# CICE-Consortium/CICE

Measured on AMD Instinct MI355X. Metric: EVP subcycle cell-updates/sec (gx1 fp64), higher is better.
Workload: dtype f64

## Files before the change

### cice_amd/csrc/evp_host_resident.cpp

```cpp
#include "evp_host.h"
#include "rim_plan.h"

namespace evp_host {

bool tripole_seam() { return (S.n_seam + S.n_pole + S.n_late) > 0 || S.plan.tail > 0 || !S.plan.fin_dst.empty(); }

static bool tfold_image(size_t k)
{
    if (!S.plan.tfold) return false;
    const int dst = S.plan.local_dst[k];
    const int b = dst / (int)S.plane, r = dst % (int)S.plane, j = r / S.d.nx_block + 1, i = r % S.d.nx_block + 1;
    return i >= S.ilo[b] && i <= S.ihi[b] && j >= S.jlo[b] && j <= S.jhi[b];
}

bool resident_possible(bool with_peers)
{
    if (!with_peers && !S.plan.peers.empty()) return false;
    if (S.plan.tfold) {
        for (const HaloPeer &p : S.plan.peers)
            for (int k = 0; k < p.n_ghost_recv; ++k) {
                const int dst = p.recv_dst[k];
                const int b = dst / (int)S.plane, r = dst % (int)S.plane, j = r / S.d.nx_block + 1, i = r % S.d.nx_block + 1;
                if (i >= S.ilo[b] && i <= S.ihi[b] && j >= S.jlo[b] && j <= S.jhi[b]) return false;
            }
// ... 176 lines not shown
        }
    if (!S.res_err) {
        if (S.mem.alloc(S.res_err, 8)) return -1;
        HIPC(hipMemset(S.res_err, 0, 8 * sizeof(int)));
    }
    return 0;
}

bool resident2_fits(bool remote)
{
    struct Key { int dev, logw, strict, capm; unsigned fl; bool remote; long cap; };
    static std::vector<Key> known;
    const unsigned fl = S.flags & S.flags_allowed & ~(EVP_F_WATER_IS_OCN | EVP_F_TBU_ZERO);
    long cap = -1;
    for (const Key &k : known)
        if (k.dev == S.device && k.logw == S.res2_logw && k.strict == (S.prm.strict != 0) && k.capm == cap_mode() && k.fl == fl && k.remote == remote)
            cap = k.cap;
    if (cap < 0) {
        hipDeviceProp_t prop;
        if (hipGetDeviceProperties(&prop, S.device) != hipSuccess) return false;
        const int per_cu = std::min(evp_resident2_max_blocks_per_cu(S.prm.strict != 0, cap_mode(), fl, S.res2_logw, remote), 8);
        cap = (long)per_cu * prop.multiProcessorCount;
        known.push_back(Key{S.device, S.res2_logw, S.prm.strict != 0, cap_mode(), fl, remote, cap});
    }
    const int need = (remote || !S.plan.peers.empty() || S.res2_order_stale || !S.res2_order || S.res2_order_for != S.res2_logw)
                         ? S.res2_ntiles : std::max(S.res2_nlive, 1);
    return S.res2_ntiles > 0 && (long)need * 10 <= cap * 9;
}


bool resident2_fits_now()
{
    if (!S.plan.peers.empty() || S.res_remote) return true;
    if (resident_tables() || resident2_order()) { g_err.clear(); return false; }
    return resident2_fits(false);
}

int resident2_order()
{
    if (S.res2_order && !S.res2_order_stale && S.res2_order_for == S.res2_logw) return 0;
    const int W = 1 << S.res2_logw, H = 256 / W;
    int gx, gy;
    evp_resident_geometry(S.max_ni, S.max_nj, S.res2_logw, &gx, &gy);
    const int ntiles = gx * gy * S.d.nblocks, nx = S.d.nx_block;
    const bool permuted = !S.res2_cls_h.empty() && S.res2_logw == 4;
    std::vector<int> cost((size_t)ntiles);
    std::vector<uint8_t> live((size_t)ntiles, 1);
    std::vector<uint8_t> perm(permuted ? (size_t)ntiles * 256 : 0), late(permuted ? (size_t)ntiles : 0),
                         nact(permuted ? (size_t)ntiles : 0), nlt(permuted ? (size_t)ntiles : 0);
    bool coop_ok = permuted;
    const bool rim = permuted && S.d.nblocks == 1;
    std::vector<uint8_t> perm_rim(rim ? (size_t)ntiles * 256 : 0), uperm(rim ? (size_t)ntiles * 256 : 0), nact_rim(rim ? (size_t)ntiles : 0);
    bool rimu_ok = rim;
    for (int t = 0; t < ntiles; ++t) {
        const int b = t / (gx * gy), bx = (t % (gx * gy)) % gx, by = (t % (gx * gy)) / gx;
        const int i0 = S.ilo[b] + bx * (W - 1), j0 = S.jlo[b] + by * (H - 1);
        auto ice = [&](int pos) -> bool {
            const int i = i0 + (pos & (W - 1)), j = j0 + pos / W;
            if (i > S.ihi[b] + 1 || j > S.jhi[b] + 1) return false;
            return (S.hmask[b * S.plane + (size_t)(j - 1) * nx + (i - 1)] & 3u) != 0;
        };
        int n = 0, waves = 0;
        if (permuted) {
            const uint8_t *cl = &S.res2_cls_h[(size_t)t * 256];
            uint8_t *pm = &perm[(size_t)t * 256];
            int k = 0, nlate = 0;
            for (int pass = 0; pass < 3; ++pass)
                for (int pos = 0; pos < 256; ++pos) {
                    const bool on = cl[pos] != 0 && ice(pos);
                    const int which = on ? (cl[pos] == 2 ? 0 : 1) : 2;
                    if (which != pass) continue;
                    pm[k++] = (uint8_t)pos;
                    if (pass == 0) ++nlate;
                    if (pass < 2) ++n;
                }
            waves = (n + 63) / 64;
            nact[t] = (uint8_t)waves;
            late[t] = (uint8_t)std::min(4, (std::max(nlate, S.res2_cnt_h[t]) + 63) / 64);
            nlt[t] = (uint8_t)std::min(n, 64);
            if (nlate > 64) coop_ok = false;
            if (rim) {
                uint8_t icep[256], uown[256], upub[256];
                for (int pos = 0; pos < 256; ++pos) {
                    const int i = i0 + (pos & (W - 1)), j = j0 + pos / W;
                    icep[pos] = ice(pos);
                    uown[pos] = (pos & (W - 1)) < W - 1 && pos / W < H - 1 && i <= S.ihi[b] && j <= S.jhi[b];
                    upub[pos] = uown[pos] && S.res2_pubimg_h[b * S.plane + (size_t)(j - 1) * nx + (i - 1)];
                }
                rim_plan::Tile rt;
                rim_plan::tile(cl, icep, uown, upub, rt);
                std::copy(rt.perm, rt.perm + 256, &perm_rim[(size_t)t * 256]);
                std::copy(rt.uperm, rt.uperm + 256, &uperm[(size_t)t * 256]);
                nact_rim[t] = (uint8_t)rt.nact;
                if (!rt.ok || late[t] > 1) rimu_ok = false;
                waves = std::max(waves, rt.nact);
            }
        } else {
            int wave_on[4] = {0, 0, 0, 0};
            for (int pos = 0; pos < 256; ++pos)
                if (ice(pos)) { ++n; wave_on[pos >> 6] = 1; }
            waves = wave_on[0] + wave_on[1] + wave_on[2] + wave_on[3];
        }
        cost[t] = 1024 * waves + n;
        const bool no_ucell = i0 > S.ihi[b] || j0 > S.jhi[b];
        live[t] = !no_ucell && (n > 0 || S.res2_always_h[t] || !S.plan.peers.empty()) ? 1 : 0;
        if (no_ucell && env_test("CICE_EVP_HIP_RES_DEBUG") && (std::atoi(env_test("CICE_EVP_HIP_RES_DEBUG")) & 512)) live[t] = 1;
// ... 257 lines not shown
```

### cice_amd/csrc/evp_resident2.hip

```cpp
#include <hip/hip_runtime.h>
#include <stdint.h>
#include <algorithm>
#include <type_traits>

#ifdef CICE_EVP_HIP_TESTING
#define RES_DBG(R) ((R).dbg)
#define RES_PROF(R) ((R).prof != nullptr)
#else
#define RES_DBG(R) 0
#define RES_PROF(R) false
#endif

#include "evp_math.h"

namespace {

constexpr int RTY = 4;

typedef unsigned v4u __attribute__((ext_vector_type(4)));

__device__ __forceinline__ void st_rec2(void *p, v4u a, v4u b)
{
    asm volatile("global_store_dwordx4 %0, %1, off sc1\n\tglobal_store_dwordx4 %0, %2, off offset:16 sc1"
                 :
// ... 40 lines not shown
    const unsigned long long bits = (unsigned long long)__double_as_longlong(x);
    v4u r;
    r.x = tag; r.y = (unsigned)bits; r.z = (unsigned)(bits >> 32); r.w = tag;
    return r;
}
__device__ __forceinline__ double unpack_rec(v4u r)
{
    return __longlong_as_double((long long)(((unsigned long long)r.z << 32) | r.y));
}

template <int CTRL>
__device__ __forceinline__ double quad_perm(double v)
{
    const long long b = __double_as_longlong(v);
    const int lo = __builtin_amdgcn_update_dpp(0, (int)(b & 0xffffffffll), CTRL, 0xf, 0xf, false);
    const int hi = __builtin_amdgcn_update_dpp(0, (int)(b >> 32), CTRL, 0xf, 0xf, false);
    return __longlong_as_double(((long long)hi << 32) | (unsigned)lo);
}
constexpr int QP_X1 = 0xB1, QP_X2 = 0x4E, QP_X3 = 0x1B;

template <bool STRICT, int CAP, int LOGW, bool REMOTE, bool COOP = false, bool LEAN = false, bool RIMU = false>
__global__ __launch_bounds__(64 * RTY, REMOTE ? 2 : 3) void evp_resident2_tile(EvpArgs A, EvpResident2 R)
{
    static_assert(!COOP || (STRICT && CAP == 3 && LOGW == 4), "COOP: 16 x 16 tiles, strict build, default scalars");
    static_assert(!LEAN || (!REMOTE && !COOP && LOGW == 4), "LEAN: one rank, 16 x 16 tiles, one thread per rim cell");
    static_assert(!RIMU || LEAN, "RIMU: a schedule of the lean loop");
    using MM = Math<STRICT>;
#ifdef CICE_EVP_HIP_TESTING
    constexpr bool RANGE = LEAN;
#else
    constexpr bool RANGE = LEAN && EVP_RES2_RANGE_DEFAULT;
#endif
    using POL = std::conditional_t<RANGE, std::conditional_t<RIMU, evp_range::RangeMathLazy, evp_range::RangeMath>, evp_range::LibMath>;
    using POLE = std::conditional_t<RANGE, evp_range::RangeMath, evp_range::LibMath>;
    constexpr int W = 1 << LOGW;
    constexpr int H = 256 / W;
    constexpr int LW = W + 1;
    constexpr int NUV = ((H + 1) * LW + 7) & ~7;
    constexpr bool PERM = (LOGW == 4);
    constexpr int NSTR = RIMU ? 8 : PERM ? 6 : 4;
    constexpr int SW = PERM ? W + 1 : W;
    constexpr int SP = SW * H;
    extern __shared__ __attribute__((aligned(16))) double smem[];
    double *s_str = smem;
    double *s_tc = smem + NSTR * SP;
    double *s_u = s_tc + 4 * 256;
    double *s_v = s_u + NUV;
    double *s_uc = s_v + NUV;
    double *s_rc = nullptr, *s_r04 = nullptr;
    __shared__ int s_bad;

    __shared__ int s_chunk[4], s_simd[4], s_cu;
    __shared__ int s_slot[4];

    const int tx = threadIdx.x, ty = threadIdx.y;
    const int t = ty * 64 + tx;
    const int tile = R.order ? R.order[blockIdx.x] : (int)blockIdx.x;
    bool no_ucell;
    {
        const int pb = A.gx * A.gy;
        const int4 rb = A.blk[tile / pb];
        no_ucell = rb.x + ((tile % pb) % A.gx) * (W - 1) > rb.y || rb.z + ((tile % pb) / A.gx) * (H - 1) > rb.w;
        if (no_ucell && !(RES_DBG(R) & 512)) return;
    }
    int tq = t;
    int cu_rank = 0;
    if (PERM && R.cuload && !(RES_DBG(R) & 64)) {
        const int wave = t >> 6;
        if ((t & 63) == 0) {
            unsigned hw, xcc;
            asm volatile("s_getreg_b32 %0, hwreg(HW_REG_HW_ID)" : "=s"(hw));
            asm volatile("s_getreg_b32 %0, hwreg(HW_REG_XCC_ID)" : "=s"(xcc));
            s_simd[wave] = (int)((hw >> 4) & 3u);
            if (wave == 0) s_cu = (int)(((xcc & 7u) << 8) | ((hw >> 8) & 0xffu));
        }
        __syncthreads();
        if (t == 0) {
            int *L = R.cuload + 8 * s_cu;
            const int nact = R.nact[tile];
            int chunk_of[4] = {0, 1, 2, 3};
            unsigned spins = 0;
            bool locked = false;
            while (spins++ < 200000u) {
                if (atomicCAS(&L[0], 0, 1) == 0) { locked = true; break; }
                __builtin_amdgcn_s_sleep(2);
            }
            if (locked) {
                int ld[4];
                const int stamp = __hip_atomic_load(&L[1], __ATOMIC_RELAXED, __HIP_MEMORY_SCOPE_AGENT);
                const bool fresh = stamp != (int)R.tag_base;
#pragma unroll
                for (int q = 0; q < 4; ++q)
                    ld[q] = fresh ? 0 : __hip_atomic_load(&L[2 + q], __ATOMIC_RELAXED, __HIP_MEMORY_SCOPE_AGENT);
                const int rank = fresh ? 0 : __hip_atomic_load(&L[6], __ATOMIC_RELAXED, __HIP_MEMORY_SCOPE_AGENT);
                s_simd[0] |= rank << 8;
                bool used[4] = {false, false, false, false};
                for (int ck = 0; ck < 4; ++ck) {
                    int best = -1;
                    for (int w = 0; w < 4; ++w) {
                        if (used[w]) continue;
                        if (best < 0 || ld[s_simd[w] & 3] < ld[s_simd[best] & 3]) best = w;
                    }
                    used[best] = true;
                    chunk_of[best] = ck;
                    if (ck < nact) ld[s_simd[best] & 3] += 1;
                }
#pragma unroll
                for (int q = 0; q < 4; ++q) __hip_atomic_store(&L[2 + q], ld[q], __ATOMIC_RELAXED, __HIP_MEMORY_SCOPE_AGENT);
                __hip_atomic_store(&L[6], rank + 1, __ATOMIC_RELAXED, __HIP_MEMORY_SCOPE_AGENT);
                __hip_atomic_store(&L[1], (int)R.tag_base, __ATOMIC_RELAXED, __HIP_MEMORY_SCOPE_AGENT);
                asm volatile("s_waitcnt vmcnt(0)" ::: "memory");
                __hip_atomic_store(&L[0], 0, __ATOMIC_RELAXED, __HIP_MEMORY_SCOPE_AGENT);
            }
#pragma unroll
            for (int w = 0; w < 4; ++w) s_chunk[w] = chunk_of[w];
        }
        __syncthreads();
        tq = s_chunk[wave] * 64 + (t & 63);
        cu_rank = s_simd[0] >> 8;
    }
    const int pos = PERM ? (int)R.perm[tile * 256 + tq] : t;
    const int tcol = pos & (W - 1);
    const int trow = pos >> LOGW;
    const int sp = trow * SW + tcol;
    const int late_waves = PERM ? (int)R.late_waves[tile] : 4;
    const bool split = PERM && late_waves <= 1 && !(RES_DBG(R) & 32);
    if ((RES_DBG(R) & 16) && tile == 1 && !R.dry) return;
    const int per_blk = A.gx * A.gy;
    const int bz = tile / per_blk;
    const int bx = (tile % per_blk) % A.gx;
    const int by = (tile % per_blk) / A.gx;
    const int4 r = A.blk[bz];
    const int i0 = r.x + bx * (W - 1), j0 = r.z + by * (H - 1);
    const int i = i0 + tcol;
    const int j = j0 + trow;
    const int nx = A.nx, ny = A.ny;
    const int cb = bz * (int)A.plane;
    const int c = cb + (j - 1) * nx + (i - 1);
    const int li = (trow + 1) * LW + (tcol + 1);
    const int upos = RIMU ? (int)R.uperm[tile * 256 + tq] : pos;
    const int ucol = upos & (W - 1), urow = upos >> LOGW;
    const int ui = RIMU ? i0 + ucol : i, uj = RIMU ? j0 + urow : j;
    const int cu = RIMU ? cb + (uj - 1) * nx + (ui - 1) : c;
    const int uli = RIMU ? (urow + 1) * LW + (ucol + 1) : li;
    const int usp = RIMU ? urow * SW + ucol : sp;
    const unsigned flags = A.flags;
    const bool water = !LEAN && !(flags & EVP_F_WATER_IS_OCN);
    const bool tbu = !LEAN && !(flags & EVP_F_TBU_ZERO);
    if (COOP) {
        s_rc = s_uc + (8 + (water ? 2 : 0) + (tbu ? 1 : 0)) * 256;
        s_r04 = s_rc + 10 * 64;
    }

    const bool inT = (i <= r.y + 1) && (j <= r.w + 1);
    unsigned m = 0;
    if (inT) m = A.mask[c];
    const bool actT = inT && (m & 1u);
    const bool ownU = (ucol < W - 1) && (urow < H - 1) && (ui <= r.y) && (uj <= r.w);
    unsigned mU = m;
    if (RIMU) mU = ownU ? A.mask[cu] : 0u;
    const bool isU = ownU && (mU & 2u);
    const bool own = (tcol < W - 1 || i == r.y + 1) && (trow < H - 1 || j == r.w + 1);
    const bool pub = ownU && (R.pubmap[cu] != 0);
    const int par0 = R.par0;
    const int nlate = COOP ? (int)R.nlate[tile] : 0;
    const bool rim_owner = COOP && tq < nlate;
    const bool actN = actT && !rim_owner;
    const int g = t >> 2, qc = t & 3;
    const bool quad = COOP && g < nlate;
    int gc = 0;
    unsigned g_vel = 0, g_out = 0;
    bool gown = false;
    double sr0 = 0.0, sr1 = 0.0, sr2 = 0.0;
    if (quad) {
        const int gpos = (int)R.perm[tile * 256 + g];
        const int gcol = gpos & (W - 1), grow = gpos >> LOGW;
        const int gi = i0 + gcol, gj = j0 + grow;
        gc = cb + (gj - 1) * nx + (gi - 1);
        gown = (gcol < W - 1 || gi == r.y + 1) && (grow < H - 1 || gj == r.w + 1);
        const int gli = (grow + 1) * LW + (gcol + 1);
        const int ij = gli, im = gli - 1, jm = gli - LW, mm = gli - LW - 1;
        const int g_oa = qc == 0 ? ij : qc == 1 ? im : qc == 2 ? mm : jm;
        const int g_ob = qc == 0 ? im : qc == 1 ? ij : qc == 2 ? jm : mm;
        const int g_od = qc == 0 ? jm : qc == 1 ? mm : qc == 2 ? im : ij;
        g_vel = (unsigned)g_oa | ((unsigned)g_ob << 10) | ((unsigned)g_od << 20);
        const int gsp = grow * SW + gcol;
        const int off04 = (int)(s_r04 - s_str);
        const int g_ox = qc == 0 ? off04 + g : (qc == 1 ? 4 : qc == 2 ? 2 : 0) * SP + gsp;
        const int g_oy = qc == 0 ? off04 + 64 + g : (qc == 1 ? 5 : qc == 2 ? 3 : 1) * SP + gsp;
        g_out = (unsigned)g_ox | ((unsigned)g_oy << 16);
        sr0 = R.tab[R.cur0 * 12 + qc][gc];
        sr1 = R.tab[R.cur0 * 12 + 4 + qc][gc];
        sr2 = R.tab[R.cur0 * 12 + 8 + qc][gc];
        if (qc == 0) {
            typename MM::SI b;
            b.dxT = A.dxT[gc]; b.dyT = A.dyT[gc];
// ... 393 lines not shown
                        give_up_note(3, k, seam_partner, ra.x, tag);
                        ok = false;
                        break;
                    }
                    __builtin_amdgcn_s_sleep(1);
                }
                if (ok) {
                    const double pu = unpack_rec(ra), pv = unpack_rec(rb);
                    if (seam_role == 1) {
                        u_own = 0.5 * (u_own + isign * pu);
                        v_own = 0.5 * (v_own + isign * pv);
                    } else {
                        u_own = isign * (0.5 * (pu + isign * u_own));
                        v_own = isign * (0.5 * (pv + isign * v_own));
                    }
                }
            }
        }
        if (isU || isSeam) { s_u[li] = u_own; s_v[li] = v_own; }
        if (LEAN && ownU) {
            const unsigned tag = want + 1u;
            if (pub) st_rec2_s(wr, own_off, pack_rec(u_own, tag), pack_rec(v_own, tag));
            if (img0 >= 0) st_rec2_s(wr, img_off0, pack_rec(img_sg0 * u_own, tag), pack_rec(img_sg0 * v_own, tag));
            if (img1 >= 0) st_rec2_s(wr, img_off1, pack_rec(img_sg1 * u_own, tag), pack_rec(img_sg1 * v_own, tag));
            if (img2 >= 0) st_rec2_s(wr, img_off2, pack_rec(img_sg2 * u_own, tag), pack_rec(img_sg2 * v_own, tag));
        } else if (ownU && !published) {
            const unsigned tag = want + 1u;
            if (pub) st_rec2(wr + 2 * (size_t)c, pack_rec(u_own, tag), pack_rec(v_own, tag));
            if (img0 >= 0) { const double sg = (img0 & 1) ? -1.0 : 1.0; st_rec2(wr + 2 * (size_t)(img0 >> 1), pack_rec(sg * u_own, tag), pack_rec(sg * v_own, tag)); }
            if (img1 >= 0) { const double sg = (img1 & 1) ? -1.0 : 1.0; st_rec2(wr + 2 * (size_t)(img1 >> 1), pack_rec(sg * u_own, tag), pack_rec(sg * v_own, tag)); }
            if (img2 >= 0) { const double sg = (img2 & 1) ? -1.0 : 1.0; st_rec2(wr + 2 * (size_t)(img2 >> 1), pack_rec(sg * u_own, tag), pack_rec(sg * v_own, tag)); }
        }
        if (rpub && !published) publish_remote(((k + par0) & 1) ^ 1, u_own, v_own, want + 1u);
        EVP_STAMP(pacc3)
        if (split) __syncthreads();
        EVP_STAMP(pacc4)
        return true;
    };
    const bool rimw = RIMU && __builtin_amdgcn_readfirstlane(tq >> 6) == 0;
    typename MM::UP upre;
    auto ucell_operands = [&](typename MM::UI &q) {
        q.uold = u_own; q.vold = v_own;
        q.vrelfac = s_uc[0 * 256 + t]; q.uocn = s_uc[1 * 256 + t]; q.vocn = s_uc[2 * 256 + t];
        q.forcex = s_uc[3 * 256 + t]; q.forcey = s_uc[4 * 256 + t]; q.Umassdti = s_uc[5 * 256 + t];
        q.fm = s_uc[6 * 256 + t]; q.uarear = s_uc[7 * 256 + t];
        q.waterx = q.uocn; q.watery = q.vocn;
        q.TbU = 0.0; q.uvel_init = 0.0; q.vvel_init = 0.0;
    };
    if constexpr (RIMU) if (rimw && isU) {
        typename MM::UI q;
        ucell_operands(q);
        MM::template stepu_pre<CAP, false, POL>(A.p, q, upre, pol);
    }
    auto subcycle_rim = [&](const int k, const v4u *rd, v4u *wr) -> bool {
        const unsigned want = R.tag_base + (unsigned)k;
        const int done = k + 1;
        if ((RES_DBG(R) & 8) && (tile & 3) == 1) {
            const unsigned long long t0 = wall_clock64();
            while (wall_clock64() - t0 < 1000ull) __builtin_amdgcn_s_sleep(8);
        }
        int bad = 0;
        if (rimw) {
            bool gave = false;
            if (ring_cp >= 0 && !(RES_DBG(R) & 2)) {
                v4u ra, rb;
                unsigned spins = 0;
                for (;;) {
                    ld_rec2_s(rd, ring_off, ra, rb);
                    if ((ra.x == want && ra.w == want && rb.x == want && rb.w == want) || (RES_DBG(R) & 1)) break;
                    if (gave_up(++spins, t_wait0)) {
                        give_up_note(1, k, ring_cp, ra.x, want);
                        __hip_atomic_store(&s_bad, 1, __ATOMIC_RELAXED, __HIP_MEMORY_SCOPE_WORKGROUP);
                        gave = true;
                        break;
                    }
                    if (RES_DBG(R) & 4) __builtin_amdgcn_s_sleep(8); else __builtin_amdgcn_s_sleep(1);
                }
                s_u[ring_li] = unpack_rec(ra);
                s_v[ring_li] = unpack_rec(rb);
            }
            __builtin_amdgcn_fence(__ATOMIC_RELEASE, "wavefront");
            __builtin_amdgcn_wave_barrier();
            __builtin_amdgcn_fence(__ATOMIC_ACQUIRE, "wavefront");
            bad = __builtin_amdgcn_ballot_w64(gave) != 0;
        }
        int slots_seen = 0;
        if (rimw && !bad) {
            const int a0 = __hip_atomic_load(&s_slot[0], __ATOMIC_RELAXED, __HIP_MEMORY_SCOPE_WORKGROUP);
            const int a1 = __hip_atomic_load(&s_slot[1], __ATOMIC_RELAXED, __HIP_MEMORY_SCOPE_WORKGROUP);
            const int a2 = __hip_atomic_load(&s_slot[2], __ATOMIC_RELAXED, __HIP_MEMORY_SCOPE_WORKGROUP);
            slots_seen = __builtin_amdgcn_readfirstlane(min(a0, min(a1, a2))) >= done;
            __builtin_amdgcn_fence(__ATOMIC_ACQUIRE, "workgroup");
        }
        EVP_STAMP(pacc0)
        if (!bad) {
            if (actT) {
                double str[8];
                a.u_ij = s_u[li]; a.v_ij = s_v[li];
                a.u_im = s_u[li - 1]; a.v_im = s_v[li - 1];
                a.u_jm = s_u[li - LW]; a.v_jm = s_v[li - LW];
                a.u_mm = s_u[li - LW - 1]; a.v_mm = s_v[li - LW - 1];
                a.strength = s_tc[0 * 256 + t]; a.DminTarea = s_tc[1 * 256 + t];
                a.dxhy = s_tc[2 * 256 + t]; a.dyhx = s_tc[3 * 256 + t];
                MM::template stress<CAP, POL>(A.p, a, s, str, pol);
                s_str[0 * SP + sp] = str[2];
                s_str[1 * SP + sp] = str[5];
                s_str[2 * SP + sp] = str[3];
                s_str[3 * SP + sp] = str[7];
                s_str[4 * SP + sp] = str[1];
                s_str[5 * SP + sp] = str[6];
                s_str[6 * SP + sp] = str[0];
                s_str[7 * SP + sp] = str[4];
            }
            EVP_STAMP(pacc1)
            __builtin_amdgcn_fence(__ATOMIC_RELEASE, "workgroup");
            if (!rimw && (t & 63) == 0) __hip_atomic_store(&s_slot[(tq >> 6) - 1], done, __ATOMIC_RELAXED, __HIP_MEMORY_SCOPE_WORKGROUP);
            if (!slots_seen) {
                unsigned spins = 0;
                for (;;) {
                    const int a0 = __hip_atomic_load(&s_slot[0], __ATOMIC_RELAXED, __HIP_MEMORY_SCOPE_WORKGROUP);
                    const int a1 = __hip_atomic_load(&s_slot[1], __ATOMIC_RELAXED, __HIP_MEMORY_SCOPE_WORKGROUP);
                    const int a2 = __hip_atomic_load(&s_slot[2], __ATOMIC_RELAXED, __HIP_MEMORY_SCOPE_WORKGROUP);
                    const int lo = __builtin_amdgcn_readfirstlane(min(a0, min(a1, a2)));
                    if (lo >= done) break;
                    if (++spins > R.spin_limit) {
                        give_up_note(5, k, -1, (unsigned)lo, (unsigned)done);
                        __hip_atomic_store(&s_bad, 1, __ATOMIC_RELAXED, __HIP_MEMORY_SCOPE_WORKGROUP);
                    }
                    if ((spins & 255u) == 0 || spins > R.spin_limit)
                        bad = __builtin_amdgcn_readfirstlane(__hip_atomic_load(&s_bad, __ATOMIC_RELAXED, __HIP_MEMORY_SCOPE_WORKGROUP));
                    if (bad) break;
                    __builtin_amdgcn_s_sleep(1);
                }
            }
            __builtin_amdgcn_fence(__ATOMIC_ACQUIRE, "workgroup");
            EVP_STAMP(pacc2)
        }
        if (!bad) {
            double fin0 = 0.0, fin1 = 0.0, fin2 = 0.0, fin3 = 0.0;
            if constexpr (POL::lazy_taub) {
                typename MM::UO o;
                if (isU) {
                    typename MM::UI q;
                    ucell_operands(q);
                    q.sx0 = s_str[6 * SP + usp]; q.sx1 = s_str[4 * SP + usp + 1];
                    q.sx2 = s_str[0 * SP + usp + SW]; q.sx3 = s_str[2 * SP + usp + SW + 1];
                    q.sy0 = s_str[7 * SP + usp]; q.sy1 = s_str[1 * SP + usp + SW];
                    q.sy2 = s_str[5 * SP + usp + 1]; q.sy3 = s_str[3 * SP + usp + SW + 1];
                    if (!rimw) MM::template stepu_pre<CAP, false, POL>(A.p, q, upre, pol);
                    MM::template stepu_post<CAP, POL>(A.p, q, upre, o, pol);
                    u_own = o.u; v_own = o.v;
                }
                if (ownU) {
                    const unsigned tag = want + 1u;
                    if (pub) st_rec2_s(wr, own_off, pack_rec(u_own, tag), pack_rec(v_own, tag));
                    if (img0 >= 0) st_rec2_s(wr, img_off0, pack_rec(img_sg0 * u_own, tag), pack_rec(img_sg0 * v_own, tag));
                    if (img1 >= 0) st_rec2_s(wr, img_off1, pack_rec(img_sg1 * u_own, tag), pack_rec(img_sg1 * v_own, tag));
                    if (img2 >= 0) st_rec2_s(wr, img_off2, pack_rec(img_sg2 * u_own, tag), pack_rec(img_sg2 * v_own, tag));
                }
                if (isU) {
                    s_u[uli] = u_own; s_v[uli] = v_own;
                    if (k == R.ndte - 1 && !R.dry) {
                        R.tab[24][cu] = o.strintx; R.tab[25][cu] = o.strinty;
                        R.tab[26][cu] = -u_own * upre.Cb; R.tab[27][cu] = -v_own * upre.Cb;
                    }
                }
            } else {
            if (isU) {
                typename MM::UI q;
                typename MM::UO o;
                ucell_operands(q);
                q.sx0 = s_str[6 * SP + usp]; q.sx1 = s_str[4 * SP + usp + 1];
                q.sx2 = s_str[0 * SP + usp + SW]; q.sx3 = s_str[2 * SP + usp + SW + 1];
                q.sy0 = s_str[7 * SP + usp]; q.sy1 = s_str[1 * SP + usp + SW];
                q.sy2 = s_str[5 * SP + usp + 1]; q.sy3 = s_str[3 * SP + usp + SW + 1];
                if (!rimw) MM::template stepu_pre<CAP, false, POL>(A.p, q, upre, pol);
                MM::template stepu_post<CAP, POL>(A.p, q, upre, o, pol);
                u_own = o.u; v_own = o.v;
                fin0 = o.strintx; fin1 = o.strinty; fin2 = o.taubx; fin3 = o.tauby;
            }
            if (ownU) {
                const unsigned tag = want + 1u;
                if (pub) st_rec2_s(wr, own_off, pack_rec(u_own, tag), pack_rec(v_own, tag));
                if (img0 >= 0) st_rec2_s(wr, img_off0, pack_rec(img_sg0 * u_own, tag), pack_rec(img_sg0 * v_own, tag));
                if (img1 >= 0) st_rec2_s(wr, img_off1, pack_rec(img_sg1 * u_own, tag), pack_rec(img_sg1 * v_own, tag));
                if (img2 >= 0) st_rec2_s(wr, img_off2, pack_rec(img_sg2 * u_own, tag), pack_rec(img_sg2 * v_own, tag));
            }
            if (isU) {
                s_u[uli] = u_own; s_v[uli] = v_own;
                if (k == R.ndte - 1 && !R.dry) {
                    R.tab[24][cu] = fin0; R.tab[25][cu] = fin1;
                    R.tab[26][cu] = fin2; R.tab[27][cu] = fin3;
                }
            }
            }
            EVP_STAMP(pacc3)
        }
        __syncthreads();
        EVP_STAMP(pacc4)
        if (s_bad) return false;
        if (rimw && isU) {
            typename MM::UI q;
            ucell_operands(q);
            MM::template stepu_pre<CAP, false, POL>(A.p, q, upre, pol);
        }
        return true;
    };
    if constexpr (RIMU) {
        const v4u *const rec_a = (const v4u *)R.rec[par0 & 1];
        v4u *const rec_b = (v4u *)R.rec[(par0 & 1) ^ 1];
        for (int k = 0; k < R.ndte; k += 2) {
            if (!subcycle_rim(k, rec_a, rec_b)) return;
            if (k + 1 == R.ndte) break;
            if (!subcycle_rim(k + 1, rec_b, (v4u *)rec_a)) return;
        }
    } else
    if (LEAN) {
        const v4u *const rec_a = (const v4u *)R.rec[par0 & 1];
        v4u *const rec_b = (v4u *)R.rec[(par0 & 1) ^ 1];
        for (int k = 0; k < R.ndte; k += 2) {
            if (!subcycle(k, rec_a, rec_b)) return;
            if (k + 1 == R.ndte) break;
            if (!subcycle(k + 1, rec_b, (v4u *)rec_a)) return;
        }
    } else {
        for (int k = 0; k < R.ndte; ++k)
            if (!subcycle(k, (const v4u *)R.rec[(k + par0) & 1], (v4u *)R.rec[((k + par0) & 1) ^ 1])) return;
    }
#undef EVP_STAMP
    if (prof && (t & 63) == 0) {
        unsigned long long *o = R.prof + ((size_t)tile * 4 + (tq >> 6)) * 8;
        o[0] = pacc0; o[1] = pacc1; o[2] = pacc2; o[3] = pacc3; o[4] = pacc4;
        o[5] = (unsigned long long)cu_rank | ((unsigned long long)(PERM && R.cuload ? s_cu : 0) << 8) | ((unsigned long long)(s_simd[t >> 6] & 3) << 24);
        unsigned long long nlib = 0;
        if constexpr (POL::ranged) nlib = pol.nlib;
        o[6] = (unsigned long long)(t >> 6) | (nlib << 8); o[7] = (unsigned long long)R.nact[tile];
    }
    if (REMOTE && ring_remote) {
        v4u ra, rb;
        const v4u *rd = (const v4u *)R.rec[(R.ndte + par0) & 1];
        const bool ok = poll_remote(rd + 2 * (size_t)ring_cp, R.tag_base + (unsigned)R.ndte, ra, rb);
        if (ok && !R.dry) {
#pragma unroll
            for (int b = 0; b < 2; ++b) { R.u[b][ring_cp] = unpack_rec(ra); R.v[b][ring_cp] = unpack_rec(rb); }
        }
    }

    if (!R.dry) {
        if (actN && own) {
#pragma unroll
            for (int k = 0; k < 12; ++k) {
                R.tab[k][c] = s[k];
                R.tab[12 + k][c] = s[k];
            }
        }
        if (quad && gown) {
            R.tab[qc][gc] = sr0; R.tab[12 + qc][gc] = sr0;
            R.tab[4 + qc][gc] = sr1; R.tab[16 + qc][gc] = sr1;
            R.tab[8 + qc][gc] = sr2; R.tab[20 + qc][gc] = sr2;
        }
        if (isU || isSeam) {
#pragma unroll
            for (int b = 0; b < 2; ++b) {
                double *uu = R.u[b], *vv = R.v[b];
                uu[cu] = u_own; vv[cu] = v_own;
                if (img0 >= 0) { const double sg = (img0 & 1) ? -1.0 : 1.0; uu[img0 >> 1] = sg * u_own; vv[img0 >> 1] = sg * v_own; }
                if (img1 >= 0) { const double sg = (img1 & 1) ? -1.0 : 1.0; uu[img1 >> 1] = sg * u_own; vv[img1 >> 1] = sg * v_own; }
                if (img2 >= 0) { const double sg = (img2 & 1) ? -1.0 : 1.0; uu[img2 >> 1] = sg * u_own; vv[img2 >> 1] = sg * v_own; }
// ... 154 lines not shown
```

### cice_amd/csrc/rim_plan.cpp

```cpp
#include "rim_plan.h"

#include <algorithm>

namespace rim_plan {

namespace {

int missing_ucells(int pos, const uint8_t *uown, const bool *in_lu, int *which)
{
    const int r = pos / W, c = pos % W;
    int n = 0;
    for (int dr = 0; dr < 2; ++dr)
        for (int dc = 0; dc < 2; ++dc) {
            const int ur = r - dr, uc = c - dc;
            if (ur < 0 || uc < 0 || ur > W - 2 || uc > W - 2) continue;
            const int u = ur * W + uc;
            if (uown[u] && !in_lu[u]) which[n++] = u;
        }
    return n;
}

}

void tile(const uint8_t *cls, const uint8_t *ice, const uint8_t *uown, const uint8_t *upub, Tile &o)
// ... 98 lines not shown
        for (int pi = 1; pi <= nx; ++pi) {
            if (pi >= ilo && pi <= ihi && pj >= jlo && pj <= jhi) continue;
            int si, sj;
            if (ghost_src(pi, pj, si, sj)) pub[(size_t)(sj - 1) * nx + (si - 1)] = 1;
        }
    for (int pass = 0; pass < 2; ++pass)
        for (int by = 0; by < B.gy; ++by)
            for (int bx = 0; bx < B.gx; ++bx) {
                const int t = by * B.gx + bx;
                const int i0 = ilo + bx * (W - 1), j0 = jlo + by * (H - 1);
                if (pass == 1) {
                    uint8_t *ice = &B.ice[(size_t)t * NPOS], *uown = &B.uown[(size_t)t * NPOS], *upub = &B.upub[(size_t)t * NPOS];
                    for (int pos = 0; pos < NPOS; ++pos) {
                        const int tcol = pos % W, trow = pos / W, i = i0 + tcol, j = j0 + trow;
                        if (i > ihi + 1 || j > jhi + 1) continue;
                        const size_t cp = (size_t)(j - 1) * nx + (i - 1);
                        ice[pos] = (mask[cp] & 3u) != 0;
                        uown[pos] = tcol < W - 1 && trow < H - 1 && i <= ihi && j <= jhi;
                        upub[pos] = uown[pos] && pub[cp];
                    }
                    tile(&B.cls[(size_t)t * NPOS], ice, uown, upub, B.tiles[(size_t)t]);
                    continue;
                }
                std::fill(ringli.begin(), ringli.end(), 0);
                for (int trow = 0; trow < H; ++trow)
                    for (int tcol = 0; tcol < W; ++tcol) {
                        const int i = i0 + tcol, j = j0 + trow;
                        if (i > ihi + 1 || j > jhi + 1) continue;
                        for (int q = 0; q < 4; ++q) {
                            const int di = -(q & 1), dj = -(q >> 1);
                            const int pc = tcol + di, pr = trow + dj, pi = i + di, pj = j + dj;
                            const bool interior = pi >= ilo && pi <= ihi && pj >= jlo && pj <= jhi;
                            if (interior && pc >= 0 && pc <= W - 2 && pr >= 0 && pr <= H - 2) continue;
                            int si, sj;
                            if (!interior && !ghost_src(pi, pj, si, sj)) continue;
                            ringli[(size_t)(pr + 1) * LW + (pc + 1)] = 1;
                            if (interior) pub[(size_t)(pj - 1) * nx + (pi - 1)] = 1;
                            else pub[(size_t)(sj - 1) * nx + (si - 1)] = 1;
                        }
                    }
                for (int trow = 0; trow < H; ++trow)
                    for (int tcol = 0; tcol < W; ++tcol) {
                        const int i = i0 + tcol, j = j0 + trow;
                        const bool computed = i <= ihi + 1 && j <= jhi + 1;
                        const int li = (trow + 1) * LW + (tcol + 1);
                        const bool late = computed && (ringli[li] || ringli[li - 1] || ringli[li - LW] || ringli[li - LW - 1]);
                        B.cls[(size_t)t * NPOS + trow * W + tcol] = late ? 2 : computed ? 1 : 0;
                    }
            }
    B.ok = true;
    for (const Tile &tl : B.tiles) B.ok = B.ok && tl.ok;
}

}
```

### cice_amd/csrc/rim_plan.h

```cpp
#pragma once
#include <cstdint>
#include <vector>

namespace rim_plan {

constexpr int W = 16, NPOS = 256, NONE = 255;

struct Tile {
    uint8_t perm[NPOS];
    uint8_t uperm[NPOS];
    int n_lt, n_lu;
    int nact;
    int nact_packed;
    bool ok;
};

void tile(const uint8_t *cls, const uint8_t *ice, const uint8_t *uown, const uint8_t *upub, Tile &out);

struct Block {
    int gx, gy;
    std::vector<uint8_t> cls, ice, uown, upub;
    std::vector<Tile> tiles;
    bool ok;
};
void block(int ni, int nj, bool cyclic_ew, bool cyclic_ns, const uint8_t *mask, Block &out);

}
```

Measured before the change: 33.37 billion.

## Split RIMU subcycle into rim-wave and interior-wave loops with counter slot sync

Splits the RIMU resident subcycle into separate code paths for the rim wave (which polls ring records and publishes images) and the interior waves (stress, a shared slot counter, then the u-cell update), removing runtime branches on rimw. The three per-wave slot flags become a single atomic fetch_add counter. Image offsets are staged in LDS and image signs are assumed positive, guarded by a new host check (records_fit) that disables RIMU when any sign is negative or the grid is too large. Interior waves now run stepu_pre after the barrier instead of overlapping it, which shortens the critical path for rim waves but may add serial work to interior waves.

```diff
diff --git a/cice_amd/csrc/evp_host_resident.cpp b/cice_amd/csrc/evp_host_resident.cpp
--- a/cice_amd/csrc/evp_host_resident.cpp
+++ b/cice_amd/csrc/evp_host_resident.cpp
@@ -252,6 +252,7 @@
     const bool rim = permuted && S.d.nblocks == 1;
     std::vector<uint8_t> perm_rim(rim ? (size_t)ntiles * 256 : 0), uperm(rim ? (size_t)ntiles * 256 : 0), nact_rim(rim ? (size_t)ntiles : 0);
     bool rimu_ok = rim;
+    if (rimu_ok) rimu_ok = rim_plan::records_fit(S.plan.local_sign.data(), S.plan.local_sign.size(), (size_t)S.plane * S.d.nblocks);
     for (int t = 0; t < ntiles; ++t) {
         const int b = t / (gx * gy), bx = (t % (gx * gy)) % gx, by = (t % (gx * gy)) / gx;
         const int i0 = S.ilo[b] + bx * (W - 1), j0 = S.jlo[b] + by * (H - 1);
diff --git a/cice_amd/csrc/evp_resident2.hip b/cice_amd/csrc/evp_resident2.hip
--- a/cice_amd/csrc/evp_resident2.hip
+++ b/cice_amd/csrc/evp_resident2.hip
@@ -116,6 +116,7 @@
 
     __shared__ int s_chunk[4], s_simd[4], s_cu;
     __shared__ int s_slot[4];
+    __shared__ unsigned s_img[3][64];
 
     const int tx = threadIdx.x, ty = threadIdx.y;
     const int t = ty * 64 + tx;
@@ -200,12 +201,12 @@
     const int j = j0 + trow;
     const int nx = A.nx, ny = A.ny;
     const int cb = bz * (int)A.plane;
-    const int c = cb + (j - 1) * nx + (i - 1);
+    int c = cb + (j - 1) * nx + (i - 1);
     const int li = (trow + 1) * LW + (tcol + 1);
     const int upos = RIMU ? (int)R.uperm[tile * 256 + tq] : pos;
     const int ucol = upos & (W - 1), urow = upos >> LOGW;
     const int ui = RIMU ? i0 + ucol : i, uj = RIMU ? j0 + urow : j;
-    const int cu = RIMU ? cb + (uj - 1) * nx + (ui - 1) : c;
+    int cu = RIMU ? cb + (uj - 1) * nx + (ui - 1) : c;
     const int uli = RIMU ? (urow + 1) * LW + (ucol + 1) : li;
     const int usp = RIMU ? urow * SW + ucol : sp;
     const unsigned flags = A.flags;
@@ -705,168 +706,222 @@
         ucell_operands(q);
         MM::template stepu_pre<CAP, false, POL>(A.p, q, upre, pol);
     }
-    auto subcycle_rim = [&](const int k, const v4u *rd, v4u *wr) -> bool {
-        const unsigned want = R.tag_base + (unsigned)k;
-        const int done = k + 1;
+    static_assert((-1 >> 1) == -1, "img >> 1 of 'no image' stays -1");
+    static_assert(!(RIMU && REMOTE), "RIMU: images come from the push table only, filled img0 first");
+    constexpr unsigned R_NOIMG = 32u * (unsigned)(-1 >> 1), R_NORING = 0xffffffffu;
+    unsigned r_own = own_off, r_ring = ring_cp >= 0 ? ring_off : R_NORING;
+    int r_sp = sp, r_usp = usp;
+    if constexpr (RIMU) {
+        static_assert(!RIMU || LW == SW, "RIMU: li == sp + LW + 1");
+        asm volatile("" : "+v"(r_own), "+v"(r_ring), "+v"(r_sp), "+v"(r_usp));
+        if (rimw) { s_img[0][t & 63] = img_off0; s_img[1][t & 63] = img_off1; s_img[2][t & 63] = img_off2; }
+    }
+    const bool has_img = RIMU && rimw && img0 >= 0;
+    const int r_li = r_sp + LW + 1, r_uli = r_usp + LW + 1;
+    auto slots_at = [&]() -> int {
+        return __builtin_amdgcn_readfirstlane(__hip_atomic_load(&s_slot[0], __ATOMIC_RELAXED, __HIP_MEMORY_SCOPE_WORKGROUP));
+    };
+    auto res_leave = [&]() {
+        __hip_atomic_store(&s_bad, 1, __ATOMIC_RELAXED, __HIP_MEMORY_SCOPE_WORKGROUP);
+        __syncthreads();
+    };
+    auto slot_spin = [&](const int k, const int done) -> bool {
+        unsigned spins = 0;
+        for (;;) {
+            const int lo = slots_at();
+            if (lo >= done) return true;
+            if (++spins > R.spin_limit) {
+                give_up_note(5, k, -1, (unsigned)lo, (unsigned)done);
+                res_leave();
+                return false;
+            }
+            if ((spins & 255u) == 0 &&
+                __builtin_amdgcn_readfirstlane(__hip_atomic_load(&s_bad, __ATOMIC_RELAXED, __HIP_MEMORY_SCOPE_WORKGROUP))) {
+                __syncthreads();
+                return false;
+            }
+            __builtin_amdgcn_s_sleep(1);
+        }
+    };
+    auto lag_hook = [&]() {
         if ((RES_DBG(R) & 8) && (tile & 3) == 1) {
             const unsigned long long t0 = wall_clock64();
             while (wall_clock64() - t0 < 1000ull) __builtin_amdgcn_s_sleep(8);
         }
-        int bad = 0;
-        if (rimw) {
-            bool gave = false;
-            if (ring_cp >= 0 && !(RES_DBG(R) & 2)) {
-                v4u ra, rb;
-                unsigned spins = 0;
-                for (;;) {
-                    ld_rec2_s(rd, ring_off, ra, rb);
-                    if ((ra.x == want && ra.w == want && rb.x == want && rb.w == want) || (RES_DBG(R) & 1)) break;
-                    if (gave_up(++spins, t_wait0)) {
-                        give_up_note(1, k, ring_cp, ra.x, want);
-                        __hip_atomic_store(&s_bad, 1, __ATOMIC_RELAXED, __HIP_MEMORY_SCOPE_WORKGROUP);
-                        gave = true;
-                        break;
-                    }
-                    if (RES_DBG(R) & 4) __builtin_amdgcn_s_sleep(8); else __builtin_amdgcn_s_sleep(1);
-                }
-                s_u[ring_li] = unpack_rec(ra);
-                s_v[ring_li] = unpack_rec(rb);
-            }
-            __builtin_amdgcn_fence(__ATOMIC_RELEASE, "wavefront");
-            __builtin_amdgcn_wave_barrier();
-            __builtin_amdgcn_fence(__ATOMIC_ACQUIRE, "wavefront");
-            bad = __builtin_amdgcn_ballot_w64(gave) != 0;
-        }
-        int slots_seen = 0;
-        if (rimw && !bad) {
-            const int a0 = __hip_atomic_load(&s_slot[0], __ATOMIC_RELAXED, __HIP_MEMORY_SCOPE_WORKGROUP);
-            const int a1 = __hip_atomic_load(&s_slot[1], __ATOMIC_RELAXED, __HIP_MEMORY_SCOPE_WORKGROUP);
-            const int a2 = __hip_atomic_load(&s_slot[2], __ATOMIC_RELAXED, __HIP_MEMORY_SCOPE_WORKGROUP);
-            slots_seen = __builtin_amdgcn_readfirstlane(min(a0, min(a1, a2))) >= done;
-            __builtin_amdgcn_fence(__ATOMIC_ACQUIRE, "workgroup");
-        }
-        EVP_STAMP(pacc0)
-        if (!bad) {
-            if (actT) {
-                double str[8];
-                a.u_ij = s_u[li]; a.v_ij = s_v[li];
-                a.u_im = s_u[li - 1]; a.v_im = s_v[li - 1];
-                a.u_jm = s_u[li - LW]; a.v_jm = s_v[li - LW];
-                a.u_mm = s_u[li - LW - 1]; a.v_mm = s_v[li - LW - 1];
-                a.strength = s_tc[0 * 256 + t]; a.DminTarea = s_tc[1 * 256 + t];
-                a.dxhy = s_tc[2 * 256 + t]; a.dyhx = s_tc[3 * 256 + t];
-                MM::template stress<CAP, POL>(A.p, a, s, str, pol);
-                s_str[0 * SP + sp] = str[2];
-                s_str[1 * SP + sp] = str[5];
-                s_str[2 * SP + sp] = str[3];
-                s_str[3 * SP + sp] = str[7];
-                s_str[4 * SP + sp] = str[1];
-                s_str[5 * SP + sp] = str[6];
-                s_str[6 * SP + sp] = str[0];
-                s_str[7 * SP + sp] = str[4];
-            }
-            EVP_STAMP(pacc1)
-            __builtin_amdgcn_fence(__ATOMIC_RELEASE, "workgroup");
-            if (!rimw && (t & 63) == 0) __hip_atomic_store(&s_slot[(tq >> 6) - 1], done, __ATOMIC_RELAXED, __HIP_MEMORY_SCOPE_WORKGROUP);
-            if (!slots_seen) {
-                unsigned spins = 0;
-                for (;;) {
-                    const int a0 = __hip_atomic_load(&s_slot[0], __ATOMIC_RELAXED, __HIP_MEMORY_SCOPE_WORKGROUP);
-                    const int a1 = __hip_atomic_load(&s_slot[1], __ATOMIC_RELAXED, __HIP_MEMORY_SCOPE_WORKGROUP);
-                    const int a2 = __hip_atomic_load(&s_slot[2], __ATOMIC_RELAXED, __HIP_MEMORY_SCOPE_WORKGROUP);
-                    const int lo = __builtin_amdgcn_readfirstlane(min(a0, min(a1, a2)));
-                    if (lo >= done) break;
-                    if (++spins > R.spin_limit) {
-                        give_up_note(5, k, -1, (unsigned)lo, (unsigned)done);
-                        __hip_atomic_store(&s_bad, 1, __ATOMIC_RELAXED, __HIP_MEMORY_SCOPE_WORKGROUP);
-                    }
-                    if ((spins & 255u) == 0 || spins > R.spin_limit)
-                        bad = __builtin_amdgcn_readfirstlane(__hip_atomic_load(&s_bad, __ATOMIC_RELAXED, __HIP_MEMORY_SCOPE_WORKGROUP));
-                    if (bad) break;
-                    __builtin_amdgcn_s_sleep(1);
-                }
-            }
-            __builtin_amdgcn_fence(__ATOMIC_ACQUIRE, "workgroup");
-            EVP_STAMP(pacc2)
-        }
-        if (!bad) {
-            double fin0 = 0.0, fin1 = 0.0, fin2 = 0.0, fin3 = 0.0;
-            if constexpr (POL::lazy_taub) {
-                typename MM::UO o;
-                if (isU) {
-                    typename MM::UI q;
-                    ucell_operands(q);
-                    q.sx0 = s_str[6 * SP + usp]; q.sx1 = s_str[4 * SP + usp + 1];
-                    q.sx2 = s_str[0 * SP + usp + SW]; q.sx3 = s_str[2 * SP + usp + SW + 1];
-                    q.sy0 = s_str[7 * SP + usp]; q.sy1 = s_str[1 * SP + usp + SW];
-                    q.sy2 = s_str[5 * SP + usp + 1]; q.sy3 = s_str[3 * SP + usp + SW + 1];
-                    if (!rimw) MM::template stepu_pre<CAP, false, POL>(A.p, q, upre, pol);
-                    MM::template stepu_post<CAP, POL>(A.p, q, upre, o, pol);
-                    u_own = o.u; v_own = o.v;
-                }
-                if (ownU) {
-                    const unsigned tag = want + 1u;
-                    if (pub) st_rec2_s(wr, own_off, pack_rec(u_own, tag), pack_rec(v_own, tag));
-                    if (img0 >= 0) st_rec2_s(wr, img_off0, pack_rec(img_sg0 * u_own, tag), pack_rec(img_sg0 * v_own, tag));
-                    if (img1 >= 0) st_rec2_s(wr, img_off1, pack_rec(img_sg1 * u_own, tag), pack_rec(img_sg1 * v_own, tag));
-                    if (img2 >= 0) st_rec2_s(wr, img_off2, pack_rec(img_sg2 * u_own, tag), pack_rec(img_sg2 * v_own, tag));
-                }
-                if (isU) {
-                    s_u[uli] = u_own; s_v[uli] = v_own;
-                    if (k == R.ndte - 1 && !R.dry) {
-                        R.tab[24][cu] = o.strintx; R.tab[25][cu] = o.strinty;
-                        R.tab[26][cu] = -u_own * upre.Cb; R.tab[27][cu] = -v_own * upre.Cb;
+    };
+    auto ucell_partials = [&](typename MM::UI &q) {
+        q.sx0 = s_str[6 * SP + r_usp]; q.sx1 = s_str[4 * SP + r_usp + 1];
+        q.sx2 = s_str[0 * SP + r_usp + SW]; q.sx3 = s_str[2 * SP + r_usp + SW + 1];
+        q.sy0 = s_str[7 * SP + r_usp]; q.sy1 = s_str[1 * SP + r_usp + SW];
+        q.sy2 = s_str[5 * SP + r_usp + 1]; q.sy3 = s_str[3 * SP + r_usp + SW + 1];
+    };
+    auto store_last = [&](const typename MM::UO &o) {
+        int cl = (int)(r_own >> 5);
+        asm volatile("" : "+v"(cl));
+        R.tab[24][cl] = o.strintx; R.tab[25][cl] = o.strinty;
+        if constexpr (POL::lazy_taub) { R.tab[26][cl] = -u_own * upre.Cb; R.tab[27][cl] = -v_own * upre.Cb; }
+        else { R.tab[26][cl] = o.taubx; R.tab[27][cl] = o.tauby; }
+    };
+    auto rim_subcycle = [&](const int k, const v4u *rd, v4u *wr) -> bool {
+        const unsigned want = R.tag_base + (unsigned)k;
+        const int done = 3 * (k + 1);
+        lag_hook();
+        if (!(RES_DBG(R) & 2)) {
+            v4u ra, rb;
+            bool pend = r_ring != R_NORING;
+            unsigned spins = 0;
+            for (;;) {
+                if (pend) {
+                    ld_rec2_s(rd, r_ring, ra, rb);
+                    if ((ra.x == want && ra.w == want && rb.x == want && rb.w == want) || (RES_DBG(R) & 1)) {
+                        s_u[ring_li] = unpack_rec(ra);
+                        s_v[ring_li] = unpack_rec(rb);
+                        pend = false;
                     }
                 }
-            } else {
-            if (isU) {
-                typename MM::UI q;
-                typename MM::UO o;
-                ucell_operands(q);
-                q.sx0 = s_str[6 * SP + usp]; q.sx1 = s_str[4 * SP + usp + 1];
-                q.sx2 = s_str[0 * SP + usp + SW]; q.sx3 = s_str[2 * SP + usp + SW + 1];
-                q.sy0 = s_str[7 * SP + usp]; q.sy1 = s_str[1 * SP + usp + SW];
-                q.sy2 = s_str[5 * SP + usp + 1]; q.sy3 = s_str[3 * SP + usp + SW + 1];
-                if (!rimw) MM::template stepu_pre<CAP, false, POL>(A.p, q, upre, pol);
-                MM::template stepu_post<CAP, POL>(A.p, q, upre, o, pol);
-                u_own = o.u; v_own = o.v;
-                fin0 = o.strintx; fin1 = o.strinty; fin2 = o.taubx; fin3 = o.tauby;
-            }
-            if (ownU) {
-                const unsigned tag = want + 1u;
-                if (pub) st_rec2_s(wr, own_off, pack_rec(u_own, tag), pack_rec(v_own, tag));
-                if (img0 >= 0) st_rec2_s(wr, img_off0, pack_rec(img_sg0 * u_own, tag), pack_rec(img_sg0 * v_own, tag));
-                if (img1 >= 0) st_rec2_s(wr, img_off1, pack_rec(img_sg1 * u_own, tag), pack_rec(img_sg1 * v_own, tag));
-                if (img2 >= 0) st_rec2_s(wr, img_off2, pack_rec(img_sg2 * u_own, tag), pack_rec(img_sg2 * v_own, tag));
-            }
-            if (isU) {
-                s_u[uli] = u_own; s_v[uli] = v_own;
-                if (k == R.ndte - 1 && !R.dry) {
-                    R.tab[24][cu] = fin0; R.tab[25][cu] = fin1;
-                    R.tab[26][cu] = fin2; R.tab[27][cu] = fin3;
+                if (__builtin_amdgcn_ballot_w64(pend) == 0) break;
+                ++spins;
+                if (spins > R.spin_limit ||
+                    ((spins & 255u) == 0 && __builtin_amdgcn_readfirstlane(__hip_atomic_load(R.err, __ATOMIC_RELAXED, __HIP_MEMORY_SCOPE_AGENT)) != 0)) {
+                    if (pend) give_up_note(1, k, (int)(r_ring >> 5), ra.x, want);
+                    res_leave();
+                    return false;
                 }
-            }
-            }
-            EVP_STAMP(pacc3)
-        }
+                if (RES_DBG(R) & 4) __builtin_amdgcn_s_sleep(8); else __builtin_amdgcn_s_sleep(1);
+            }
+        }
+        __builtin_amdgcn_fence(__ATOMIC_RELEASE, "wavefront");
+        __builtin_amdgcn_wave_barrier();
+        __builtin_amdgcn_fence(__ATOMIC_ACQUIRE, "wavefront");
+        const bool slots_seen = slots_at() >= done;
+        __builtin_amdgcn_fence(__ATOMIC_ACQUIRE, "workgroup");
+        EVP_STAMP(pacc0)
+        if (actT) {
+            double str[8];
+            a.u_ij = s_u[r_li]; a.v_ij = s_v[r_li];
+            a.u_im = s_u[r_li - 1]; a.v_im = s_v[r_li - 1];
+            a.u_jm = s_u[r_li - LW]; a.v_jm = s_v[r_li - LW];
+            a.u_mm = s_u[r_li - LW - 1]; a.v_mm = s_v[r_li - LW - 1];
+            a.strength = s_tc[0 * 256 + t]; a.DminTarea = s_tc[1 * 256 + t];
+            a.dxhy = s_tc[2 * 256 + t]; a.dyhx = s_tc[3 * 256 + t];
+            MM::template stress<CAP, POL>(A.p, a, s, str, pol);
+            s_str[0 * SP + r_sp] = str[2];
+            s_str[1 * SP + r_sp] = str[5];
+            s_str[2 * SP + r_sp] = str[3];
+            s_str[3 * SP + r_sp] = str[7];
+            s_str[4 * SP + r_sp] = str[1];
+            s_str[5 * SP + r_sp] = str[6];
+            s_str[6 * SP + r_sp] = str[0];
+            s_str[7 * SP + r_sp] = str[4];
+        }
+        EVP_STAMP(pacc1)
+        if (!slots_seen) {
+            if (!slot_spin(k, done)) return false;
+            __builtin_amdgcn_fence(__ATOMIC_ACQUIRE, "workgroup");
+        }
+        EVP_STAMP(pacc2)
+        unsigned o0 = R_NOIMG, o1 = R_NOIMG, o2 = R_NOIMG;
+        if (has_img) { o0 = s_img[0][t & 63]; o1 = s_img[1][t & 63]; o2 = s_img[2][t & 63]; }
+        typename MM::UO o;
+        if (isU) {
+            typename MM::UI q;
+            ucell_operands(q);
+            ucell_partials(q);
+            MM::template stepu_post<CAP, POL>(A.p, q, upre, o, pol);
+            u_own = o.u; v_own = o.v;
+        }
+        if (ownU) {
+            const unsigned tag = want + 1u;
+            const v4u gu = pack_rec(u_own, tag), gv = pack_rec(v_own, tag);
+            if (pub) st_rec2_s(wr, r_own, gu, gv);
+            if (has_img) {
+                st_rec2_s(wr, o0, gu, gv);
+                if (o1 != R_NOIMG) {
+                    st_rec2_s(wr, o1, gu, gv);
+                    if (o2 != R_NOIMG) st_rec2_s(wr, o2, gu, gv);
+                }
+            }
+        }
+        if (isU) {
+            s_u[r_uli] = u_own; s_v[r_uli] = v_own;
+            if (k == R.ndte - 1 && !R.dry) store_last(o);
+        }
+        EVP_STAMP(pacc3)
         __syncthreads();
         EVP_STAMP(pacc4)
         if (s_bad) return false;
-        if (rimw && isU) {
+        if (isU) {
             typename MM::UI q;
             ucell_operands(q);
             MM::template stepu_pre<CAP, false, POL>(A.p, q, upre, pol);
         }
         return true;
     };
+    auto interior_subcycle = [&](const int k) -> bool {
+        const int done = 3 * (k + 1);
+        lag_hook();
+        EVP_STAMP(pacc0)
+        if (actT) {
+            double str[8];
+            a.u_ij = s_u[r_li]; a.v_ij = s_v[r_li];
+            a.u_im = s_u[r_li - 1]; a.v_im = s_v[r_li - 1];
+            a.u_jm = s_u[r_li - LW]; a.v_jm = s_v[r_li - LW];
+            a.u_mm = s_u[r_li - LW - 1]; a.v_mm = s_v[r_li - LW - 1];
+            a.strength = s_tc[0 * 256 + t]; a.DminTarea = s_tc[1 * 256 + t];
+            a.dxhy = s_tc[2 * 256 + t]; a.dyhx = s_tc[3 * 256 + t];
+            MM::template stress<CAP, POL>(A.p, a, s, str, pol);
+            s_str[0 * SP + r_sp] = str[2];
+            s_str[1 * SP + r_sp] = str[5];
+            s_str[2 * SP + r_sp] = str[3];
+            s_str[3 * SP + r_sp] = str[7];
+            s_str[4 * SP + r_sp] = str[1];
+            s_str[5 * SP + r_sp] = str[6];
+            s_str[6 * SP + r_sp] = str[0];
+            s_str[7 * SP + r_sp] = str[4];
+        }
+        EVP_STAMP(pacc1)
+        __builtin_amdgcn_fence(__ATOMIC_RELEASE, "workgroup");
+        if ((t & 63) == 0) __hip_atomic_fetch_add(&s_slot[0], 1, __ATOMIC_RELAXED, __HIP_MEMORY_SCOPE_WORKGROUP);
+        if (!slot_spin(k, done)) return false;
+        __builtin_amdgcn_fence(__ATOMIC_ACQUIRE, "workgroup");
+        EVP_STAMP(pacc2)
+        if (isU) {
+            typename MM::UI q;
+            typename MM::UO o;
+            ucell_operands(q);
+            ucell_partials(q);
+            MM::template stepu_pre<CAP, false, POL>(A.p, q, upre, pol);
+            MM::template stepu_post<CAP, POL>(A.p, q, upre, o, pol);
+            u_own = o.u; v_own = o.v;
+            s_u[r_uli] = u_own; s_v[r_uli] = v_own;
+            if (k == R.ndte - 1 && !R.dry) store_last(o);
+        }
+        EVP_STAMP(pacc3)
+        __syncthreads();
+        EVP_STAMP(pacc4)
+        return !s_bad;
+    };
     if constexpr (RIMU) {
         const v4u *const rec_a = (const v4u *)R.rec[par0 & 1];
         v4u *const rec_b = (v4u *)R.rec[(par0 & 1) ^ 1];
-        for (int k = 0; k < R.ndte; k += 2) {
-            if (!subcycle_rim(k, rec_a, rec_b)) return;
-            if (k + 1 == R.ndte) break;
-            if (!subcycle_rim(k + 1, rec_b, (v4u *)rec_a)) return;
-        }
+        if (rimw) {
+            for (int k = 0; k < R.ndte; k += 2) {
+                if (!rim_subcycle(k, rec_a, rec_b)) return;
+                if (k + 1 == R.ndte) break;
+                if (!rim_subcycle(k + 1, rec_b, (v4u *)rec_a)) return;
+            }
+        } else {
+            for (int k = 0; k < R.ndte; ++k)
+                if (!interior_subcycle(k)) return;
+        }
+        asm volatile("" : "+v"(r_own), "+v"(r_sp));
+        const unsigned r_img0 = rimw ? s_img[0][t & 63] : R_NOIMG, r_img1 = rimw ? s_img[1][t & 63] : R_NOIMG, r_img2 = rimw ? s_img[2][t & 63] : R_NOIMG;
+        c = cb + (j0 + r_sp / SW - 1) * nx + (i0 + r_sp % SW - 1);
+        cu = (int)(r_own >> 5);
+        if (isU) { u_own = s_u[r_uli]; v_own = s_v[r_uli]; }
+        img0 = r_img0 == R_NOIMG ? -1 : (int)(r_img0 >> 5) << 1;
+        img1 = r_img1 == R_NOIMG ? -1 : (int)(r_img1 >> 5) << 1;
+        img2 = r_img2 == R_NOIMG ? -1 : (int)(r_img2 >> 5) << 1;
     } else
     if (LEAN) {
         const v4u *const rec_a = (const v4u *)R.rec[par0 & 1];
diff --git a/cice_amd/csrc/rim_plan.cpp b/cice_amd/csrc/rim_plan.cpp
--- a/cice_amd/csrc/rim_plan.cpp
+++ b/cice_amd/csrc/rim_plan.cpp
@@ -174,4 +174,12 @@
     for (const Tile &tl : B.tiles) B.ok = B.ok && tl.ok;
 }
 
+bool records_fit(const int8_t *sign, size_t n, size_t ncell)
+{
+    if (ncell > ((size_t)1 << 27)) return false;
+    for (size_t k = 0; k < n; ++k)
+        if (sign[k] < 0) return false;
+    return true;
 }
+
+}
diff --git a/cice_amd/csrc/rim_plan.h b/cice_amd/csrc/rim_plan.h
--- a/cice_amd/csrc/rim_plan.h
+++ b/cice_amd/csrc/rim_plan.h
@@ -1,4 +1,5 @@
 #pragma once
+#include <cstddef>
 #include <cstdint>
 #include <vector>
 
@@ -25,4 +26,6 @@
 };
 void block(int ni, int nj, bool cyclic_ew, bool cyclic_ns, const uint8_t *mask, Block &out);
 
+bool records_fit(const int8_t *sign, size_t n, size_t ncell);
+
 }
```

After: 33.79 billion (median of 6 runs). 1.3% higher.
